# jl6017/AutoURDF

Measured on AMD Instinct MI355X. Metric: registered frames/sec (N=4096 pts, K=20 clusters), higher is better.
Workload: dtype f32

## Files before the change

autourdf_amd/csrc/nn_l1.h:

```cpp
#pragma once
#include <type_traits>
#include "creg_dev.h"

namespace creg {

constexpr int NN_TCH = 4096;
constexpr int NN_BLOCK = 512;
typedef float nn_f2 __attribute__((ext_vector_type(2)));

struct NnEpilogueNone {
    __device__ __forceinline__ void finish(int, int, float, float*) const {}
    __device__ __forceinline__ void shift(int) {}
};

template <int QW, typename IdxT, typename Epi>
__device__ __forceinline__ void nn_l1_block(
    const float* A, int na, int sa, const float* B, int nb, int sb,
    float* __restrict__ dA, IdxT* __restrict__ iA, float* __restrict__ dB, IdxT* __restrict__ iB,
    int blocksA, Epi& epi, int bx) {
    extern __shared__ __attribute__((aligned(16))) char smem_raw[];
    float* sX = (float*)smem_raw;
    __shared__ float s_part[NN_BLOCK / 64];
    const int tid = threadIdx.x, lane = tid & 63;
    const int wave = __builtin_amdgcn_readfirstlane(tid >> 6);
// ... 73 lines not shown
#pragma unroll
        for (int e = 3; e >= 0; --e) {
            const int j = bgrp[u] + 64 * e;
            const float d = l1_dist(qx[u], qy[u], qz[u], rx[u][e], ry[u][e], rz[u][e]);
            if (bgrp[u] >= 0 && j < nt && d == best[u]) bi = j;
        }
        float v = best[u]; int i = bi;
        wave_argmin_fast(v, i);
        if (lane == u) { mv = v; mi = i; mqx = qx[u]; mqy = qy[u]; mqz = qz[u]; }
    }
    if (lane < QW && q0 + lane < nq) {
        if (dO) { dO[q0 + lane] = mv; iO[q0 + lane] = (IdxT)mi; }
        if constexpr (!std::is_same<Epi, NnEpilogueNone>::value) {
            float tx, ty, tz;
            if (in_lds) { tx = sX[mi]; ty = sX[padded0 + mi]; tz = sX[2 * padded0 + mi]; }
            else { const float* p = T + (size_t)mi * st; tx = p[0]; ty = p[1]; tz = p[2]; }
            epi(dir, q0 + lane, mi, mv, mqx, mqy, mqz, tx, ty, tz, acc);
        }
    }
    if constexpr (!std::is_same<Epi, NnEpilogueNone>::value) {
        acc = wave_sum_fast(acc);
        if (lane == 0) s_part[wave] = acc;
        __syncthreads();
        if (tid == 0) {
            float s = 0.f;
#pragma unroll
            for (int w = 0; w < NN_BLOCK / 64; ++w) s += s_part[w];
            epi.finish(dir, blk, s, nullptr);
        }
    }
}

struct NnBlocks { const float4* ts4; const float* tbox; int nblk; const int* nblk_dev; };

template <int NB, int PPL, typename Epi, bool STOP = false, bool NBDEV = false>
__device__ __forceinline__ void nn_l1_block_pruned(const float* Q, int nq, int sq, NnBlocks tb, int dir, Epi& epi, int blk,
                                                   const int* stop_flag = nullptr, const float* T = nullptr, int st = 0) {
    constexpr int QW = 4;
    int stop = 0;
    if constexpr (STOP) stop = *stop_flag;
    __shared__ float s_partp[NN_BLOCK / 64];
    const int tid = threadIdx.x, lane = tid & 63;
    const int wave = __builtin_amdgcn_readfirstlane(tid >> 6);
    const int q0 = (blk * (NN_BLOCK / 64) + wave) * QW;
    int nblk = tb.nblk;
    if constexpr (NBDEV) nblk = *tb.nblk_dev;
    float lox[NB], loy[NB], loz[NB], hix[NB], hiy[NB], hiz[NB];
#pragma unroll
    for (int g = 0; g < NB; ++g) {
        const float* bx = tb.tbox + (NBDEV ? 64 * g + lane : min(64 * g + lane, nblk - 1));
        constexpr int BP = 64 * NB;
        lox[g] = bx[0]; loy[g] = bx[BP]; loz[g] = bx[2 * BP]; hix[g] = bx[3 * BP]; hiy[g] = bx[4 * BP]; hiz[g] = bx[5 * BP];
    }
    float qx[QW], qy[QW], qz[QW], lb[QW][NB], bd[QW], tx[QW], ty[QW], tz[QW], wb[QW];
    int bi[QW];
    unsigned long long pend[QW][NB];
#pragma unroll
    for (int u = 0; u < QW; ++u) {
        const int qi = min(q0 + u, nq - 1);
        qx[u] = Q[(size_t)qi * sq]; qy[u] = Q[(size_t)qi * sq + 1]; qz[u] = Q[(size_t)qi * sq + 2];
    }
    if constexpr (STOP || NBDEV) {
        stop = __builtin_amdgcn_readfirstlane(stop); nblk = __builtin_amdgcn_readfirstlane(nblk);
#pragma unroll
        for (int u = 0; u < QW; ++u) {
            qx[u] = __int_as_float(__builtin_amdgcn_readfirstlane(__float_as_int(qx[u])));
            qy[u] = __int_as_float(__builtin_amdgcn_readfirstlane(__float_as_int(qy[u])));
            qz[u] = __int_as_float(__builtin_amdgcn_readfirstlane(__float_as_int(qz[u])));
        }
    }
#pragma unroll
    for (int u = 0; u < QW; ++u) {
        float lm = INFINITY;
#pragma unroll
        for (int g = 0; g < NB; ++g) {
            const float ex = fmaxf(fmaxf(lox[g] - qx[u], qx[u] - hix[g]), 0.f);
            const float ey = fmaxf(fmaxf(loy[g] - qy[u], qy[u] - hiy[g]), 0.f);
            const float ez = fmaxf(fmaxf(loz[g] - qz[u], qz[u] - hiz[g]), 0.f);
            const float bound = (ex + ey) + ez;
            lb[u][g] = 64 * g + lane < nblk ? bound : INFINITY;
            lm = __builtin_fminf(lm, lb[u][g]);
        }
        const float m = wave_min_fast(lm);
        bool found = false;
#pragma unroll
        for (int g = 0; g < NB; ++g) {
            const unsigned long long f = __ballot(lb[u][g] == m && 64 * g + lane < nblk);
            pend[u][g] = (!found && f) ? (f & (~f + 1ull)) : 0ull;
            found = found || f != 0ull;
        }
        if (!found) pend[u][0] = 1ull;
        bd[u] = INFINITY; bi[u] = 0x7fffffff; tx[u] = ty[u] = tz[u] = 0.f; wb[u] = INFINITY;
    }
    if (stop) return;
    bool more = true;
    while (more) {
        int b[QW];
        bool act[QW];
#pragma unroll
        for (int u = 0; u < QW; ++u) {
            b[u] = 0; act[u] = false;
#pragma unroll
            for (int g = NB - 1; g >= 0; --g)
                if (pend[u][g]) { b[u] = 64 * g + __builtin_ctzll(pend[u][g]); act[u] = true; }
        }
        float4 v1[QW];
        if constexpr (PPL == 1) {
#pragma unroll
            for (int u = 0; u < QW; ++u) v1[u] = tb.ts4[(size_t)b[u] * 64 + lane];
        }
        more = false;
#pragma unroll
        for (int u = 0; u < QW; ++u) {
            if (act[u]) {
                float4 v[PPL];
                if constexpr (PPL == 1) v[0] = v1[u];
                else {
#pragma unroll
                    for (int k = 0; k < PPL; ++k) v[k] = tb.ts4[((size_t)b[u] * PPL + k) * 64 + lane];
                }
#pragma unroll
                for (int g = 0; g < NB; ++g)
                    if ((b[u] >> 6) == g && lane == (b[u] & 63)) lb[u][g] = INFINITY;
                if constexpr (PPL > 1) {
                    unsigned long long key = ((unsigned long long)__float_as_uint(bd[u]) << 32) | (unsigned)bi[u];
#pragma unroll
                    for (int k = 0; k < PPL; ++k) {
                        const float d = l1_dist(qx[u], qy[u], qz[u], v[k].x, v[k].y, v[k].z);
                        const unsigned long long kk = ((unsigned long long)__float_as_uint(d) << 32) | (unsigned)__float_as_int(v[k].w);
                        key = kk < key ? kk : key;
                    }
                    bd[u] = __uint_as_float((unsigned)(key >> 32)); bi[u] = (int)(unsigned)key;
                } else {
#pragma unroll
                    for (int k = 0; k < PPL; ++k) {
                        const float d = l1_dist(qx[u], qy[u], qz[u], v[k].x, v[k].y, v[k].z);
                        const int oi = __float_as_int(v[k].w);
                        const unsigned long long key = ((unsigned long long)__float_as_uint(bd[u]) << 32) | (unsigned)bi[u];
                        const unsigned long long kk = ((unsigned long long)__float_as_uint(d) << 32) | (unsigned)oi;
                        const bool take = kk < key;
                        bd[u] = take ? d : bd[u]; bi[u] = take ? oi : bi[u];
                        tx[u] = take ? v[k].x : tx[u]; ty[u] = take ? v[k].y : ty[u]; tz[u] = take ? v[k].z : tz[u];
                    }
                }
                wb[u] = wave_min_fast(bd[u]);
#pragma unroll
                for (int g = 0; g < NB; ++g) {
                    pend[u][g] = __ballot(lb[u][g] <= wb[u] && lb[u][g] < INFINITY);
                    more |= pend[u][g] != 0ull;
                }
            }
        }
    }
    float acc = 0.f, mv = 0.f, mqx = 0.f, mqy = 0.f, mqz = 0.f, mtx = 0.f, mty = 0.f, mtz = 0.f;
    int mi = 0;
#pragma unroll
    for (int u = 0; u < QW; ++u) {
        const int i = wave_min_fast(bd[u] == wb[u] ? bi[u] : 0x7fffffff);
        const unsigned long long win = __ballot(bd[u] == wb[u] && bi[u] == i);
        const int src = win ? __builtin_ctzll(win) : 0;
        const float fx = __int_as_float(__builtin_amdgcn_readlane(__float_as_int(tx[u]), src));
        const float fy = __int_as_float(__builtin_amdgcn_readlane(__float_as_int(ty[u]), src));
        const float fz = __int_as_float(__builtin_amdgcn_readlane(__float_as_int(tz[u]), src));
        if (lane == u) { mv = wb[u]; mi = i; mqx = qx[u]; mqy = qy[u]; mqz = qz[u]; mtx = fx; mty = fy; mtz = fz; }
    }
    if constexpr (PPL > 1) {
        if (lane < QW && q0 + lane < nq && mi != 0x7fffffff) { const float* p = T + (size_t)mi * st; mtx = p[0]; mty = p[1]; mtz = p[2]; }
    }
    if (lane < QW && q0 + lane < nq) epi(dir, q0 + lane, mi, mv, mqx, mqy, mqz, mtx, mty, mtz, acc);
    acc = wave_sum_fast(acc);
    if (lane == 0) s_partp[wave] = acc;
    __syncthreads();
    if (tid == 0) {
        float s = 0.f;
#pragma unroll
        for (int w = 0; w < NN_BLOCK / 64; ++w) s += s_partp[w];
        epi.finish(dir, blk, s, nullptr);
    }
}

__device__ __forceinline__ float row_min16(float v) {
    asm("s_nop 4\n\t"
        "v_min_f32_dpp %0, %0, %0 quad_perm:[1,0,3,2] row_mask:0xf bank_mask:0xf\n\ts_nop 1\n\t"
        "v_min_f32_dpp %0, %0, %0 quad_perm:[2,3,0,1] row_mask:0xf bank_mask:0xf\n\ts_nop 1\n\t"
        "v_min_f32_dpp %0, %0, %0 row_half_mirror row_mask:0xf bank_mask:0xf\n\ts_nop 1\n\t"
        "v_min_f32_dpp %0, %0, %0 row_mirror row_mask:0xf bank_mask:0xf\n\ts_nop 1"
        : "+v"(v));
    return v;
}
__device__ __forceinline__ float row_max16(float v) {
    asm("s_nop 4\n\t"
        "v_max_f32_dpp %0, %0, %0 quad_perm:[1,0,3,2] row_mask:0xf bank_mask:0xf\n\ts_nop 1\n\t"
        "v_max_f32_dpp %0, %0, %0 quad_perm:[2,3,0,1] row_mask:0xf bank_mask:0xf\n\ts_nop 1\n\t"
        "v_max_f32_dpp %0, %0, %0 row_half_mirror row_mask:0xf bank_mask:0xf\n\ts_nop 1\n\t"
        "v_max_f32_dpp %0, %0, %0 row_mirror row_mask:0xf bank_mask:0xf\n\ts_nop 1"
        : "+v"(v));
    return v;
}
__device__ __forceinline__ float row_sum16_f(float v) {
    CREG_DPP_STEP(v, 0xB1, 0xF);
    CREG_DPP_STEP(v, 0x4E, 0xF);
    CREG_DPP_STEP(v, 0x141, 0xF);
    CREG_DPP_STEP(v, 0x140, 0xF);
    return v;
}
__device__ __forceinline__ unsigned long long key_min_rows(unsigned long long k) {
    {   const auto hi = __builtin_amdgcn_permlane16_swap((unsigned)(k >> 32), (unsigned)(k >> 32), false, false);
        const auto lo = __builtin_amdgcn_permlane16_swap((unsigned)k, (unsigned)k, false, false);
        const unsigned long long a = ((unsigned long long)hi[0] << 32) | lo[0], b = ((unsigned long long)hi[1] << 32) | lo[1];
        k = a < b ? a : b; }
    {   const auto hi = __builtin_amdgcn_permlane32_swap((unsigned)(k >> 32), (unsigned)(k >> 32), false, false);
        const auto lo = __builtin_amdgcn_permlane32_swap((unsigned)k, (unsigned)k, false, false);
        const unsigned long long a = ((unsigned long long)hi[0] << 32) | lo[0], b = ((unsigned long long)hi[1] << 32) | lo[1];
        k = a < b ? a : b; }
    return k;
}
#ifdef CREG_NN_STATS
__device__ unsigned long long g_nn_stats[8];
#define NN_STAT(i, v) do { if (lane == 0) atomicAdd(&g_nn_stats[i], (unsigned long long)(v)); } while (0)
#else
#define NN_STAT(i, v) do { } while (0)
#endif
#ifdef CREG_NN_WAVE_STAMPS
struct NnWaveRec { unsigned long long t0, t1, t2, t3; int visits, cands, dir, blk; };
constexpr unsigned NN_WAVE_CAP = 1u << 19, NN_WAVE_SHARDS = 256, NN_WAVE_PER = NN_WAVE_CAP / NN_WAVE_SHARDS;
__device__ NnWaveRec g_nn_wave[NN_WAVE_CAP];
__device__ unsigned g_nn_wave_n[NN_WAVE_SHARDS * 32];
#define NN_WSTAMP(...) __VA_ARGS__
#else
#define NN_WSTAMP(...)
#endif
constexpr int NN_ROWQ = 16;
#ifndef NN_ROW_FIRST
#define NN_ROW_FIRST 2
#endif
#ifndef NN_ROW_BATCH
#define NN_ROW_BATCH 3
#endif
#ifndef NN_ROWS_BLOCK
#define NN_ROWS_BLOCK 256
#endif
constexpr int NN_ROW_SLOTS = (NN_ROWS_BLOCK / 64) * NN_ROWQ;

template <int NB, typename Epi, bool NBDEV, bool NQDEV>
__device__ __forceinline__ void nn_l1_rows(const float4* __restrict__ qs4, int nqblk, const int* nqblk_dev, int nqblk_host, NnBlocks tb, int dir, Epi& epi, int blk,
                                           const int* stop_flag, const float* __restrict__ T, float* __restrict__ lossp) {
    const int tid = threadIdx.x, lane = tid & 63, q = lane & 15, g = lane >> 4;
    const int wave = __builtin_amdgcn_readfirstlane(tid >> 6);
    const int grp = blk * (NN_ROWS_BLOCK / 64) + wave;
    if (grp >= 4 * nqblk_host) return;
    NN_WSTAMP(const unsigned long long ws_t0 = (unsigned long long)wall_clock64(); unsigned long long ws_t1 = 0, ws_t2 = 0; int ws_vis = 0, ws_cand = 0;)
    int stop = *stop_flag;
    int nblk = tb.nblk;
    if constexpr (NBDEV) nblk = *tb.nblk_dev;
    if constexpr (NQDEV) nqblk = *nqblk_dev;
// ... 175 lines not shown
```

autourdf_amd/csrc/train_backward.hip:

```cpp
#include <cmath>
#include <cstddef>
#include <cstring>
#include "train_dev.h"

namespace creg {

__device__ __forceinline__ TrainState advance_state(const TrainState& S, float loss, const Hyper& hy, double bc1, float bc2_sqrt) {
    TrainState N = S;
    const bool improved = loss < S.min_loss;
    N.last_loss = loss;
    N.epochs_run = S.epochs_run + 1;
    const int count = improved ? 0 : S.count + 1;
    N.min_loss = improved ? loss : S.min_loss;
    N.best_epoch = improved ? S.epochs_run : S.best_epoch;
    N.count = count;
    N.stopped = (!improved && count > hy.stop) ? 1 : S.stopped;
    if (!N.stopped) {
        N.step = S.step + 1;
        N.step_size = (float)(S.lr / bc1);
        N.bc2_sqrt = bc2_sqrt;
        const double cur = (double)loss;
        if (cur < S.sched_best * (1.0 - 1e-4)) { N.sched_best = cur; N.sched_bad = 0; }
        else N.sched_bad = S.sched_bad + 1;
        if (N.sched_bad > hy.patience) {
            const double nl = fmax(S.lr * (double)hy.factor, 0.0);
            if (S.lr - nl > 1e-8) N.lr = nl;
            N.sched_bad = 0;
        }
    }
    return N;
}

constexpr int GC_QMAX = 3;
__device__ __forceinline__ void gradc_role(const Dims& D, const Ws& W, int epoch, int nbx, int nby, int k) {
    __shared__ float red[4][14];
    __shared__ float s_loss;
    __shared__ float s_go[16];
    const int tid = threadIdx.x, lane = tid & 63, wv = tid >> 6;
    const TrainState S = W.state[epoch & 1];
    const int b0 = W.off[k], e0 = W.off[k + 1];
    const Hyper hy = *W.hyper;
    float a = tid < nbx ? W.lossp_x[tid] : 0.f, b = tid < nby ? W.lossp_y[tid] : 0.f;
    const float m2v = W.m2[16 * k + (tid & 15)];
    float sv[16];
#pragma unroll
    for (int i = 0; i < 16; ++i) sv[i] = W.head_save[16 * k + i];
    const float* h2cur = (epoch & 1) ? W.h2[1] : W.h2[0];
    float w3v[GC_QMAX][8], h2v[GC_QMAX];
#pragma unroll
    for (int q = 0; q < GC_QMAX; ++q) {
        const int o = min(q * 256 + tid, D.H2 - 1);
        const bool isA = o < D.HA;
        const float* Pc = (epoch & 1) ? W.P1 : W.P;
        const float* wb = isA ? Pc + D.oW3A + o : Pc + D.oW3B + (o - D.HA);
        const int stride = isA ? D.HA : D.HB, nj = isA ? D.OA : D.OB;
#pragma unroll
        for (int j = 0; j < 8; ++j) w3v[q][j] = wb[(size_t)min(j, nj - 1) * stride];
        h2v[q] = h2cur[(size_t)k * D.H2 + o];
    }
    asm volatile("" :: "v"(a), "v"(b), "v"(m2v), "v"(sv[0]), "v"(sv[1]), "v"(sv[2]), "v"(sv[3]), "v"(sv[4]), "v"(sv[5]), "v"(sv[6]), "v"(sv[7]),
                 "v"(sv[8]), "v"(sv[9]), "v"(sv[10]), "v"(sv[11]), "v"(sv[12]), "v"(sv[13]), "v"(sv[14]), "v"(sv[15]), "v"(b0), "v"(e0), "v"(hy.lr));
#pragma unroll
    for (int q = 0; q < GC_QMAX; ++q)
        asm volatile("" :: "v"(h2v[q]), "v"(w3v[q][0]), "v"(w3v[q][1]), "v"(w3v[q][2]), "v"(w3v[q][3]), "v"(w3v[q][4]), "v"(w3v[q][5]), "v"(w3v[q][6]),
                     "v"(w3v[q][7]));
    if (S.stopped) {
        if (k == 0 && tid == 0) {
            TrainState E = S; E.stopped = 1;
            W.state[(epoch + 1) & 1] = E;
        }
        return;
    }
    const int n_first = min(b0 + tid, D.NP - 1);
    const float4 p_first = W.pts4[n_first];
    const int4 c_first = W.cnt4[n_first];
    const int s_first = W.sgn_x[n_first];
    const float4 pr_first = W.pred4[n_first];
    for (int i = tid + 256; i < nbx; i += 256) a += W.lossp_x[i];
    for (int i = tid + 256; i < nby; i += 256) b += W.lossp_y[i];
    a = wave_sum_fast(a); b = wave_sum_fast(b);
    if (lane == 0) { red[wv][0] = a; red[wv][1] = b; }
    __syncthreads();
    if (tid == 0) {
        const float sa = ((red[0][0] + red[1][0]) + red[2][0]) + red[3][0];
        const float sb = ((red[0][1] + red[1][1]) + red[2][1]) + red[3][1];
        s_loss = sa / (float)D.NP + sb / (float)D.NT;
    }
    __syncthreads();
    const float loss = s_loss;
    TrainState N = advance_state(S, loss, hy, S.next_bc1, S.next_bc2s);
    const bool improved = loss < S.min_loss;
    if (improved) {
        for (int n = b0 + tid; n < e0; n += 256) {
            const float4 p = (n == b0 + tid) ? pr_first : W.pred4[n];
            W.best_pred[3 * (size_t)n] = p.x; W.best_pred[3 * (size_t)n + 1] = p.y; W.best_pred[3 * (size_t)n + 2] = p.z;
        }
        if (tid < 16) W.best_m[16 * k + tid] = m2v;
    }
    if (k == 0 && tid == 0) {
        N.next_bc1 = W.bc1[min(N.step + 1, D.epochs)];
        N.next_bc2s = W.bc2s[min(N.step + 1, D.epochs)];
        W.state[(epoch + 1) & 1] = N;
        W.loss_hist[S.epochs_run] = loss;
        W.lr_hist[S.epochs_run] = (float)S.lr;
        W.result[0] = N.min_loss; W.result[1] = (float)N.epochs_run; W.result[2] = (float)N.lr; W.result[3] = (float)N.best_epoch;
    }
    if (N.stopped) return;
    const float gx = 1.0f / (float)D.NP, gy = 1.0f / (float)D.NT;
    float acc[12];
#pragma unroll
    for (int i = 0; i < 12; ++i) acc[i] = 0.f;
    for (int n = b0 + tid; n < e0; n += 256) {
// ... 34 lines not shown
            float gu[4];
            quat_to_matrix_vjp(sv, G, gu);
            const float nrm = sv[4];
            if (nrm > 1e-12f) {
                const float dot = sv[0] * gu[0] + sv[1] * gu[1] + sv[2] * gu[2] + sv[3] * gu[3];
#pragma unroll
                for (int i = 0; i < 4; ++i) go[4 + i] = (gu[i] - sv[i] * dot) / nrm;
            } else {
#pragma unroll
                for (int i = 0; i < 4; ++i) go[4 + i] = gu[i] / 1e-12f;
            }
        } else {
            float gdq[8];
            dq_to_se3_vjp(sv, G, gt, gdq);
            for (int i = 0; i < 8; ++i) go[4 + i] = gdq[i];
        }
        for (int i = 0; i < 12; ++i) { W.g_out[16 * k + i] = go[i]; s_go[i] = go[i]; }
    }
    __syncthreads();
#pragma unroll
    for (int q = 0; q < GC_QMAX; ++q) {
        const int o = q * 256 + tid;
        if (o < D.H2) {
            const bool isA = o < D.HA;
            const int nj = isA ? D.OA : D.OB, gofs = isA ? 0 : 4;
            float sum = 0.f;
#pragma unroll
            for (int j = 0; j < 8; ++j) if (j < nj) sum = fmaf(s_go[gofs + j], w3v[q][j], sum);
            W.g_h2[(size_t)k * D.H2 + o] = sum * act_grad(h2v[q], D.slope);
        }
    }
}

__global__ __launch_bounds__(256) void k_gradc(Dims D, Ws W0, int epoch, int nbx, int nby, size_t bstride) {
    asm volatile("" :: "s"(W0.P), "s"(W0.P1), "s"(W0.h2[0]), "s"(W0.h2[1]), "s"(W0.head_save), "s"(W0.m2), "s"(W0.gm2), "s"(W0.pts4), "s"(W0.pred4),
                 "s"(W0.sgn_x), "s"(W0.cnt4), "s"(W0.lossp_x), "s"(W0.lossp_y), "s"(W0.g_out), "s"(W0.g_h2), "s"(W0.state), "s"(W0.bc1), "s"(W0.bc2s),
                 "s"(W0.best_m), "s"(W0.best_pred), "s"(W0.loss_hist), "s"(W0.lr_hist), "s"(W0.result), "s"(W0.off), "s"(W0.hyper),
                 "s"(D.rot), "s"(D.K), "s"(D.H2), "s"(D.HA), "s"(D.HB), "s"(D.OA), "s"(D.OB), "s"(D.NP), "s"(D.NT), "s"(D.epochs), "s"(D.slope),
                 "s"(D.oW3A), "s"(D.oW3B), "s"(epoch), "s"(nbx), "s"(nby), "s"(bstride));
    const Ws W = ws_shift(W0, blockIdx.z * bstride);
    gradc_role(D, W, epoch, nbx, nby, blockIdx.x);
}

__device__ __forceinline__ float adam_value(float p, float& mm, float& vv, float g, float step_size, float bc2_sqrt) {
    const float b1w = (float)(1.0 - 0.9), b2 = 0.999f, b2w = (float)(1.0 - 0.999);
    mm = mm + b1w * (g - mm);
    vv = vv * b2 + (b2w * g) * g;
    const float denom = sqrtf(vv) / bc2_sqrt + 1e-8f;
    return p + (-step_size * mm) / denom;
}

#ifdef CREG_BD_STAMPS
struct BdStamps {
    unsigned long long first[256], endB[256], endD[256], startB[256], startD[256];
    unsigned long long phase[2][8], blocks[2];
    int armed;
};
__device__ BdStamps g_bd_st;
#endif
constexpr int BD_THREADS = 512;
constexpr int B2_THREADS = BD_THREADS;
constexpr int B2_WAVES = B2_THREADS / 64;
constexpr int B2_CB = 16;
constexpr int B2_RB = 32;
__host__ __device__ inline int b2_smem_floats(int K, int IN, int H2) {
    return B2_WAVES * B2_RB * B2_CB + K * IN + 2 * K * B2_CB + H2 * B2_CB;
}
__device__ __forceinline__ float row_sum16(float v) {
    CREG_DPP_STEP(v, 0xB1, 0xF);
    CREG_DPP_STEP(v, 0x4E, 0xF);
    CREG_DPP_STEP(v, 0x141, 0xF);
    CREG_DPP_STEP(v, 0x140, 0xF);
    return v;
}
// ... 264 lines not shown
__global__ __launch_bounds__(BD_THREADS, 4) void k_bd(Dims D, Ws W0, int epoch, size_t bstride, int nz) {
    extern __shared__ __attribute__((aligned(16))) char smem[];
#ifdef CREG_BD_STAMPS
    const unsigned long long bd_entry = wall_clock64();
#else
    const unsigned long long bd_entry = 0;
#endif
#ifndef CREG_BD_NO_TOUCH
    asm volatile("" :: "s"(W0.P), "s"(W0.P1), "s"(W0.AM), "s"(W0.AV), "s"(W0.enc), "s"(W0.x1[0]), "s"(W0.x1[1]), "s"(W0.h2[0]), "s"(W0.h2[1]),
                 "s"(W0.g_out), "s"(W0.g_h2), "s"(W0.state), "s"(D.K), "s"(D.KP), "s"(D.IN), "s"(D.H), "s"(D.H2), "s"(D.HA), "s"(D.HB), "s"(D.OA),
                 "s"(D.OB), "s"(D.oW1), "s"(D.ob1), "s"(D.oW2), "s"(D.ob2), "s"(D.oW3A), "s"(D.ob3A), "s"(D.oW3B), "s"(D.ob3B), "s"(D.NPAR),
                 "s"(D.slope), "s"(epoch), "s"(bstride), "s"(nz));
#endif
    const int nB = D.H / B2_CB, nD = dw_blocks(D);
    int i = blockIdx.x;
    const bool roleB = i < nB * nz;
    if (!roleB) i -= nB * nz;
    const int n = roleB ? nB : nD, z = i / n, blk = i - z * n;
    const Ws W = ws_shift(W0, (size_t)z * bstride);
#ifdef CREG_BD_ONLY
    if ((CREG_BD_ONLY == 1) != roleB) return;
#endif
    if (roleB) bwd2_role<KW, X>(D, W, epoch, blk, (float*)smem, bd_entry);
    else dw_role(D, W, epoch, blk, bd_entry);
}
constexpr int BD_K_MAX_6D_512 = 193;
constexpr int BD_LDS_MAX = 160 * 1024;
static int bd_lds_bytes(const Dims& D) { return (int)sizeof(float) * b2_smem_floats(D.K, D.IN, D.H2); }
bool backward_fits(const Dims& D) {
    if (D.rot == ROT_6D && D.H == 512 && D.K > BD_K_MAX_6D_512) return false;
    return D.K * D.IN / 4 <= 8 * BD_THREADS && bd_lds_bytes(D) <= BD_LDS_MAX && D.H2 % 32 == 0 && D.H % B2_CB == 0 && D.H2 <= 256 * GC_QMAX;
}
void launch_gradc(const Dims& D, const Slice& S, size_t bstride, int epoch, hipStream_t s) {
    hipLaunchKernelGGL(k_gradc, dim3(D.K, 1, S.nz), dim3(256), 0, s, D, S.W, epoch, D.nbx, D.nby, bstride);
}
template <typename F>
static void by_bd(const Dims& D, F f) {
    by_nc(D.H, [&](auto nc) {
        constexpr int NC = decltype(nc)::value;
        if (D.IN > 64) f(k_bd<NC, 12 * NC, true>);
        else if (D.HA) f(k_bd<NC, 12 * NC>);
        else f(k_bd<NC, 8 * NC>);
    });
}
int bd_raise_lds(const Dims& D) {
    hipError_t e = hipSuccess;
    by_bd(D, [&](auto kern) { e = hipFuncSetAttribute((const void*)kern, hipFuncAttributeMaxDynamicSharedMemorySize, BD_LDS_MAX); });
    if (e != hipSuccess) {
        set_error("creg_train_plan_create: cannot raise the dynamic LDS limit of k_bd: %s", hipGetErrorString(e));
        return CREG_EHIP;
    }
    return CREG_OK;
}
void launch_bd(const Dims& D, const Slice& S, size_t bstride, int epoch, hipStream_t s) {
    const int per = D.H / B2_CB + dw_blocks(D);
    by_bd(D, [&](auto kern) { hipLaunchKernelGGL(kern, dim3(per * S.nz), dim3(BD_THREADS), bd_lds_bytes(D), s, D, S.W, epoch, bstride, S.nz); });
}

int bd_stamps_arm(bool on) {
#ifdef CREG_BD_STAMPS
    static BdStamps z;
    if (on) {
        memset(&z, 0, sizeof(z)); memset(z.first, 0xff, sizeof(z.first)); memset(z.startB, 0xff, sizeof(z.startB)); memset(z.startD, 0xff, sizeof(z.startD));
        z.armed = 1;
        CREG_HIP(hipMemcpyToSymbol(HIP_SYMBOL(g_bd_st), &z, sizeof(z)));
    } else {
        z.armed = 0;
// ... 32 lines not shown
```

autourdf_amd/csrc/train_dev.h:

```cpp
#pragma once
#include <type_traits>
#include "creg_common.h"
#include "creg_dev.h"

namespace creg {

struct Dims {
    int rot, K, KP, IN, H, HA, HB, H2, OA, OB, NP, NT, epochs;
    float slope;
    int oW1, ob1, oW2, ob2, oW3A, ob3A, oW3B, ob3B, NPAR;
    int nbx, nby;
    int nyb;
    int npb;
    int ppl;
    int nbt, nbp;
    int rows;
};

constexpr int PS_MAXB = 512;
constexpr int YS_CHUNK = 16384;

struct Hyper {
    float lr, factor;
    int patience, stop;
};

struct TrainState {
    double lr, sched_best;
    int sched_bad, count, stopped, step;
    float min_loss;
    int epochs_run, best_epoch;
    float step_size, bc2_sqrt;
    float last_loss;
    float next_bc2s;
    double next_bc1;
};

struct Ws {
    float *P, *P1, *AM, *AV;
    float *pose_in, *enc, *x1[2], *h2[2], *head_save, *m2, *gm2;
    float4 *pts4, *y4, *pred4, *ys4, *psl4, *ps4;
    float *ybox, *pbox;
    int* sb;
    int* sgn_x;
    int4* cnt4;
    float *lossp_x, *lossp_y;
    float *g_out, *g_h2;
    TrainState* state;
    double* bc1;
    float* bc2s;
// ... 75 lines not shown
```

autourdf_amd/csrc/train_engine.hip:

```cpp
#include <chrono>
#include <cstdlib>
#include <cstring>
#include <memory>
#include <vector>
#include "train_dev.h"
#include "nn_l1.h"

namespace creg {

constexpr int CHAINS_MAX = 8;

struct Plan {
    creg_train_shape shape{};
    Dims D{};
    Ws W{};
    ParamMap pm[10] = {};
    int np = 0;
    int B = 1;
    size_t bstride = 0;
    int branches = 1;
    hipGraphExec_t gexec = nullptr;
    bool graph_ready = false;
    int graph_epochs = 0;
    bool chain_streams = false;
// ... 28 lines not shown

static bool make_dims(const creg_train_shape* s, Dims* D) {
    if (!s || s->rot < 0 || s->rot > 3 || s->k < 1 || s->k > 256 || (s->hidden != 64 && s->hidden != 128 && s->hidden != 256 && s->hidden != 512) || s->epochs < 1 || s->n_pred < 1 || s->n_tgt < 1 || s->n_pred >= (1ll << 31) ||
        s->n_tgt >= (1ll << 31))
        return false;
    memset(D, 0, sizeof(*D));
    D->rot = s->rot; D->K = s->k; D->KP = (s->k + 19) / 20 * 20; D->H = s->hidden; D->NP = (int)s->n_pred; D->NT = (int)s->n_tgt; D->epochs = s->epochs;
    if (s->rot == ROT_Q) { D->IN = 56; D->HA = D->H / 2; D->HB = D->H; D->OA = 3; D->OB = 4; D->slope = 0.01f; }
    else if (s->rot == ROT_DQ) { D->IN = 64; D->HA = 0; D->HB = D->H; D->OA = 0; D->OB = 8; D->slope = 0.f; }
    else if (s->rot == ROT_6D) { D->IN = 72; D->HA = D->H / 2; D->HB = D->H; D->OA = 3; D->OB = 6; D->slope = 0.01f; }
    else { D->IN = 48; D->HA = D->H / 2; D->HB = D->H; D->OA = 3; D->OB = 3; D->slope = 0.01f; }
    D->H2 = D->HA + D->HB;
    if (!backward_fits(*D)) return false;
    int o = 0;
    D->oW1 = o; o += D->H * D->IN; D->ob1 = o; o += D->H;
    D->oW2 = o; o += D->H2 * D->H; D->ob2 = o; o += D->H2;
    D->oW3A = o; o += D->OA * D->HA; D->ob3A = o; o += D->OA;
    D->oW3B = o; o += D->OB * D->HB; D->ob3B = o; o += D->OB;
    D->NPAR = o;
    const NnGrid g = nn_grid(D->NP, D->NT, true, true, 4);
    D->nbx = g.blocksA; D->nby = g.blocksB;
    const bool rows_fit = D->NT <= YS_CHUNK && D->NP < 65535 && (D->NP + 63) / 64 + D->K <= PS_MAXB && g.qw == 4;
    const char* rows_env = getenv("CREG_NN_ROWS");
    const bool rows_pays = D->NT > 64 * 64;
    D->rows = s->nn_search == 0 && rows_fit && (rows_env ? rows_env[0] == '1' : rows_pays);
    D->ppl = (D->rows || D->NT <= 64 * 64) ? 1 : 4;
    const int BS = 64 * D->ppl;
    D->nyb = (s->nn_search != 1 && D->NT <= 4 * YS_CHUNK && g.qw == 4) ? (D->NT + BS - 1) / BS : 0;
    D->npb = (D->nyb && D->NP < 65535 && (D->NP + BS - 1) / BS + D->K <= PS_MAXB) ? (D->NP + BS - 1) / BS + D->K : 0;
    const int nt = (D->nyb + 63) / 64, np = (D->npb + 63) / 64;
    D->nbt = nt <= 1 ? 1 : (nt <= 2 ? 2 : 4);
    D->nbp = np <= 2 ? 2 : (np <= 3 ? 3 : (np <= 4 ? 4 : (np <= 5 ? 5 : (np <= 6 ? 6 : 8))));
    if (D->rows) { D->nbx = 4 * D->npb; D->nby = 4 * D->nyb; }
    return true;
}

static size_t carve(const Dims& D, char* base, Ws* W) {
    size_t o = 0;
    auto take = [&](size_t bytes) -> char* { char* r = base ? base + o : nullptr; o = align_up(o + bytes, 256); return r; };
    const size_t f = sizeof(float);
    Ws w;
    w.P = (float*)take(f * D.NPAR); w.P1 = (float*)take(f * D.NPAR); w.AM = (float*)take(f * D.NPAR); w.AV = (float*)take(f * D.NPAR);
    w.pose_in = (float*)take(f * POSE_IN * D.K); w.enc = (float*)take(f * D.K * D.IN);
    w.x1[0] = (float*)take(f * D.KP * D.H); w.x1[1] = (float*)take(f * D.KP * D.H);
    w.h2[0] = (float*)take(f * D.KP * D.H2); w.h2[1] = (float*)take(f * D.KP * D.H2); w.head_save = (float*)take(f * 16 * D.K);
    w.m2 = (float*)take(f * 16 * D.K); w.gm2 = (float*)take(f * 16 * D.K);
    w.pts4 = (float4*)take(sizeof(float4) * D.NP); w.y4 = (float4*)take(sizeof(float4) * D.NT);
    w.pred4 = (float4*)take(sizeof(float4) * D.NP);
    const size_t bs = 64 * (size_t)D.ppl;
    w.ys4 = (float4*)take(sizeof(float4) * bs * (D.nyb ? D.nyb : 1)); w.ybox = (float*)take(f * 6 * 64 * D.nbt);
    w.psl4 = (float4*)take(sizeof(float4) * bs * (D.npb ? D.npb : 1)); w.ps4 = (float4*)take(sizeof(float4) * bs * (D.npb ? D.npb : 1));
    w.pbox = (float*)take(f * 6 * 64 * D.nbp); w.sb = (int*)take(sizeof(int) * (D.K + 1));
    w.sgn_x = (int*)take(sizeof(int) * D.NP);
    w.cnt4 = (int4*)take(sizeof(int4) * D.NP);
    w.lossp_x = (float*)take(f * D.nbx); w.lossp_y = (float*)take(f * D.nby);
    w.g_out = (float*)take(f * 16 * D.KP); w.g_h2 = (float*)take(f * D.KP * D.H2);
    w.state = (TrainState*)take(sizeof(TrainState) * 2);
    w.bc1 = (double*)take(sizeof(double) * (D.epochs + 1)); w.bc2s = (float*)take(f * (D.epochs + 1));
    w.best_m = (float*)take(f * 16 * D.K); w.best_pred = (float*)take(f * 3 * D.NP);
    w.loss_hist = (float*)take(f * D.epochs); w.lr_hist = (float*)take(f * D.epochs); w.result = (float*)take(f * 4);
    w.off = (int*)take(sizeof(int) * (D.K + 1)); w.hyper = (Hyper*)take(sizeof(Hyper));
    w.ysum = (unsigned long long*)take(sizeof(unsigned long long) * 4);
    if (W) *W = w;
    return o;
}
constexpr int NKERN = 5;
// ... 406 lines not shown
```

autourdf_amd/csrc/train_nn.hip:

```cpp
#include <type_traits>
#include <vector>
#include "train_dev.h"
#include "nn_l1.h"

namespace creg {

struct EngineEpi {
    int* sgn_x; int4* cnt4; float* lossp_x; float* lossp_y;
    size_t bstride;
    const int* stopped;
    __device__ __forceinline__ void shift(int z) {
        const size_t b = (size_t)z * bstride;
        sgn_x = (int*)((char*)sgn_x + b); cnt4 = (int4*)((char*)cnt4 + b);
        lossp_x = (float*)((char*)lossp_x + b); lossp_y = (float*)((char*)lossp_y + b);
        stopped = (const int*)((const char*)stopped + b);
    }
    __device__ __forceinline__ void operator()(int dir, int q, int idx, float d, float qx, float qy, float qz,
                                               float tx, float ty, float tz, float& acc) const {
        if (dir == 0) {
            sgn_x[q] = (qx > tx ? 1 : 0) | (qy > ty ? 2 : 0) | (qz > tz ? 4 : 0);
        } else {
            atomicAdd(&cnt4[idx].x, (qx > tx) ? -1 : 1);
            atomicAdd(&cnt4[idx].y, (qy > ty) ? -1 : 1);
            atomicAdd(&cnt4[idx].z, (qz > tz) ? -1 : 1);
        }
        acc += d;
    }
    __device__ __forceinline__ void finish(int dir, int blk, float s, float*) const { (dir == 0 ? lossp_x : lossp_y)[blk] = s; }
};

template <bool P1, int PPL, int NBT, int NBP>
__global__ __launch_bounds__(NN_BLOCK) void k_nn_plan(const float* A, int na, const float* B, int nb, int blocksA,
                                                      int blocksB, EngineEpi epi, NnBlocks yb, NnBlocks pb, size_t zstride) {
    asm volatile("" :: "s"(A), "s"(na), "s"(B), "s"(nb), "s"(blocksA), "s"(blocksB), "s"(epi.sgn_x), "s"(epi.cnt4), "s"(epi.lossp_x), "s"(epi.lossp_y),
                 "s"(epi.bstride), "s"(epi.stopped), "s"(yb.ts4), "s"(yb.tbox), "s"(yb.nblk), "s"(pb.ts4), "s"(pb.tbox), "s"(pb.nblk_dev), "s"(zstride));
    const int nz = gridDim.x / (blocksA + blocksB);
    int i = blockIdx.x, z, bx;
    if (i < blocksB * nz) { z = i / blocksB; bx = blocksA + (i - z * blocksB); }
    else { i -= blocksB * nz; z = i / blocksA; bx = i - z * blocksA; }
    const size_t zb = z * zstride;
    A = (const float*)((const char*)A + zb);
    B = (const float*)((const char*)B + zb);
    yb.ts4 = (const float4*)((const char*)yb.ts4 + zb);
    yb.tbox = (const float*)((const char*)yb.tbox + zb);
    epi.shift(z);
    if (bx < blocksA) nn_l1_block_pruned<NBT, PPL, EngineEpi, true, false>(A, na, 4, yb, 0, epi, bx, epi.stopped, B, 4);
    else if constexpr (P1) {
        pb.ts4 = (const float4*)((const char*)pb.ts4 + zb);
        pb.tbox = (const float*)((const char*)pb.tbox + zb);
        pb.nblk_dev = (const int*)((const char*)pb.nblk_dev + zb);
        nn_l1_block_pruned<NBP, PPL, EngineEpi, true, true>(B, nb, 4, pb, 1, epi, bx - blocksA, epi.stopped, A, 4);
    } else nn_l1_block<4, int, EngineEpi>(A, na, 4, B, nb, 4, nullptr, nullptr, nullptr, nullptr, blocksA, epi, bx);
}

template <int NBT, int NBP>
__global__ __launch_bounds__(NN_ROWS_BLOCK) void k_nn_rows(const float* A, const float* B, int blocksA, int blocksB, EngineEpi epi, NnBlocks yb, NnBlocks pb,
                                                      size_t zstride) {
    asm volatile("" :: "s"(A), "s"(B), "s"(blocksA), "s"(blocksB), "s"(epi.sgn_x), "s"(epi.cnt4), "s"(epi.lossp_x), "s"(epi.lossp_y),
                 "s"(epi.bstride), "s"(epi.stopped), "s"(yb.ts4), "s"(yb.tbox), "s"(yb.nblk), "s"(pb.ts4), "s"(pb.tbox), "s"(pb.nblk_dev), "s"(zstride));
    const int nz = gridDim.x / (blocksA + blocksB);
    int i = blockIdx.x, z, bx;
    if (i < blocksB * nz) { z = i / blocksB; bx = blocksA + (i - z * blocksB); }
    else { i -= blocksB * nz; z = i / blocksA; bx = i - z * blocksA; }
    const size_t zb = z * zstride;
    A = (const float*)((const char*)A + zb);
    B = (const float*)((const char*)B + zb);
    yb.ts4 = (const float4*)((const char*)yb.ts4 + zb);
    yb.tbox = (const float*)((const char*)yb.tbox + zb);
    pb.ts4 = (const float4*)((const char*)pb.ts4 + zb);
    pb.tbox = (const float*)((const char*)pb.tbox + zb);
    pb.nblk_dev = (const int*)((const char*)pb.nblk_dev + zb);
    epi.shift(z);
    if (bx < blocksA) nn_l1_rows<NBT, EngineEpi, false, true>(pb.ts4, 0, pb.nblk_dev, pb.nblk, yb, 0, epi, bx, epi.stopped, B, epi.lossp_x);
    else nn_l1_rows<NBP, EngineEpi, true, false>(yb.ts4, yb.nblk, nullptr, yb.nblk, pb, 1, epi, bx - blocksA, epi.stopped, A, epi.lossp_y);
}
template <typename F>
static void by_boxes(int nbt, int nbp, F f) {
    by_value<1, 2, 4>(nbt, [&](auto t) { by_value<2, 3, 4, 5, 6, 8>(nbp, [&](auto p) { f(t, p); }); });
}

void launch_nn(const Dims& D, const Slice& S, size_t bstride, int par, hipStream_t s) {
    const Ws& W = S.W;
    const int nz = S.nz;
    const EngineEpi epi{W.sgn_x, W.cnt4, W.lossp_x, W.lossp_y, bstride, &W.state[par].stopped};
    if (D.rows) {
        const NnBlocks yb{W.ys4, W.ybox, D.nyb, nullptr}, pb{W.ps4, W.pbox, D.npb, W.sb + D.K};
        const int blocksA = cdiv(64 * D.npb, NN_ROW_SLOTS), blocksB = cdiv(64 * D.nyb, NN_ROW_SLOTS);
        const dim3 grid((blocksA + blocksB) * nz);
        by_boxes(D.nbt, D.nbp, [&](auto nbt, auto nbp) {
            hipLaunchKernelGGL((k_nn_rows<decltype(nbt)::value, decltype(nbp)::value>), grid, dim3(NN_ROWS_BLOCK), 0, s, (const float*)W.pred4, (const float*)W.y4,
                               blocksA, blocksB, epi, yb, pb, bstride);
        });
    } else if (D.nyb) {
        const NnGrid g = nn_grid(D.NP, D.NT, true, true, 4);
        const NnBlocks yb{W.ys4, W.ybox, D.nyb, nullptr}, pb{W.ps4, W.pbox, 0, W.sb + D.K};
        const dim3 grid((g.blocksA + g.blocksB) * nz);
        auto go = [&](auto kern, int smem) {
            hipLaunchKernelGGL(kern, grid, dim3(NN_BLOCK), smem, s, (const float*)W.pred4, D.NP, (const float*)W.y4, D.NT,
                               g.blocksA, g.blocksB, epi, yb, pb, bstride);
        };
        by_value<1, 4>(D.ppl, [&](auto ppl) {
            by_boxes(D.nbt, D.nbp, [&](auto nbt, auto nbp) {
                constexpr int PPL = decltype(ppl)::value, NBT = decltype(nbt)::value, NBP = decltype(nbp)::value;
                if constexpr (NBP == 2) if (!D.npb) { go(k_nn_plan<false, PPL, NBT, 2>, g.smem); return; }
                go(k_nn_plan<true, PPL, NBT, NBP>, 0);
            });
        });
    } else {
        launch_nn_l1<int>((const float*)W.pred4, D.NP, 4, (const float*)W.y4, D.NT, 4, nullptr, nullptr, nullptr, nullptr,
                          true, true, epi, s, nz, bstride, 4);
    }
}

}
using namespace creg;

#ifdef CREG_NN_STATS
extern "C" int creg_debug_nn_stats(unsigned long long* out8, int reset) {
    CREG_HIP(hipMemcpyFromSymbol(out8, HIP_SYMBOL(creg::g_nn_stats), sizeof(unsigned long long) * 8));
    if (reset) { unsigned long long z[8] = {0}; CREG_HIP(hipMemcpyToSymbol(HIP_SYMBOL(creg::g_nn_stats), z, sizeof(z))); }
    return CREG_OK;
}
#endif
// ... 24 lines not shown
```

Before: 166.5.

## Add slot-ordered NN query kernel with per-point distance write and fused gradc loss sum

Adds a new k_nn_slot path in which each wave takes its four queries in spatial slot order from the other cloud's sorted block storage. Queries that are spatially close therefore tend to visit the same target block, and the block is loaded once when all active queries agree. Each query's distance is written back into the .w of pred4/y4 rather than reduced per block into lossp partials. k_gradc then rebuilds the loss sums itself with DPP block partials, which drops the block reduction and __syncthreads from the NN kernel. The path is on by default, with an env var to opt out, and only applies for ppl==1 with both clouds boxed and small enough. It risks extra global writes and more complex control flow.

Result: slower. 137.9 (-17.2%).

```diff
diff --git a/autourdf_amd/csrc/nn_l1.h b/autourdf_amd/csrc/nn_l1.h
--- a/autourdf_amd/csrc/nn_l1.h
+++ b/autourdf_amd/csrc/nn_l1.h
@@ -129,17 +129,31 @@
 }
 
 struct NnBlocks { const float4* ts4; const float* tbox; int nblk; const int* nblk_dev; };
-
-template <int NB, int PPL, typename Epi, bool STOP = false, bool NBDEV = false>
+#ifdef CREG_NN_STATS
+__device__ unsigned long long g_nn_stats[8];
+#define NN_STAT(i, v) do { if (lane == 0) atomicAdd(&g_nn_stats[i], (unsigned long long)(v)); } while (0)
+#else
+#define NN_STAT(i, v) do { } while (0)
+#endif
+
+template <int NB, int PPL, typename Epi, bool STOP = false, bool NBDEV = false, int SLOTW = 0, bool NQDEV = false>
 __device__ __forceinline__ void nn_l1_block_pruned(const float* Q, int nq, int sq, NnBlocks tb, int dir, Epi& epi, int blk,
-                                                   const int* stop_flag = nullptr, const float* T = nullptr, int st = 0) {
+                                                   const int* stop_flag = nullptr, const float* T = nullptr, int st = 0,
+                                                   const float4* __restrict__ qs4 = nullptr, int nqblk = 0, const int* nqblk_dev = nullptr) {
     constexpr int QW = 4;
+    constexpr bool SLOT = SLOTW > 0;
+    static_assert(!SLOT || (PPL == 1 && STOP), "slot-order queries: one point per lane, with the stop flag");
     int stop = 0;
     if constexpr (STOP) stop = *stop_flag;
     __shared__ float s_partp[NN_BLOCK / 64];
     const int tid = threadIdx.x, lane = tid & 63;
     const int wave = __builtin_amdgcn_readfirstlane(tid >> 6);
-    const int q0 = (blk * (NN_BLOCK / 64) + wave) * QW;
+    const int q0 = (blk * (SLOT ? SLOTW : NN_BLOCK / 64) + wave) * QW;
+    float4 qv = make_float4(0.f, 0.f, 0.f, 0.f);
+    if constexpr (SLOT) {
+        if constexpr (NQDEV) nqblk = *nqblk_dev;
+        qv = qs4[q0 + (lane & 3)];
+    }
     int nblk = tb.nblk;
     if constexpr (NBDEV) nblk = *tb.nblk_dev;
     float lox[NB], loy[NB], loz[NB], hix[NB], hiy[NB], hiz[NB];
@@ -151,13 +165,33 @@
     }
     float qx[QW], qy[QW], qz[QW], lb[QW][NB], bd[QW], tx[QW], ty[QW], tz[QW], wb[QW];
     int bi[QW];
+    unsigned vmask = 0xFu;
+    bool lvalid = true;
     unsigned long long pend[QW][NB];
+    if constexpr (SLOT) {
+        asm volatile("" :: "v"(qv.x), "v"(qv.y), "v"(qv.z), "v"(qv.w), "v"(nblk));
+#pragma unroll
+        for (int g = 0; g < NB; ++g) asm volatile("" :: "v"(lox[g]), "v"(loy[g]), "v"(loz[g]), "v"(hix[g]), "v"(hiy[g]), "v"(hiz[g]));
+        stop = __builtin_amdgcn_readfirstlane(stop); nqblk = __builtin_amdgcn_readfirstlane(nqblk);
+        lvalid = q0 + (lane & 3) < 64 * nqblk && __float_as_int(qv.w) != 0x7fffffff;
+        vmask = (unsigned)__ballot(lvalid) & 0xFu;
+        if (stop || !vmask) return;
+        nblk = __builtin_amdgcn_readfirstlane(nblk);
+#pragma unroll
+        for (int u = 0; u < QW; ++u) {
+            qx[u] = __int_as_float(__builtin_amdgcn_readlane(__float_as_int(qv.x), u));
+            qy[u] = __int_as_float(__builtin_amdgcn_readlane(__float_as_int(qv.y), u));
+            qz[u] = __int_as_float(__builtin_amdgcn_readlane(__float_as_int(qv.z), u));
+        }
+        NN_STAT(0 + 4 * dir, 1); NN_STAT(3 + 4 * dir, __builtin_popcount(vmask));
+    } else {
 #pragma unroll
     for (int u = 0; u < QW; ++u) {
         const int qi = min(q0 + u, nq - 1);
         qx[u] = Q[(size_t)qi * sq]; qy[u] = Q[(size_t)qi * sq + 1]; qz[u] = Q[(size_t)qi * sq + 2];
     }
-    if constexpr (STOP || NBDEV) {
+    }
+    if constexpr (!SLOT && (STOP || NBDEV)) {
         stop = __builtin_amdgcn_readfirstlane(stop); nblk = __builtin_amdgcn_readfirstlane(nblk);
 #pragma unroll
         for (int u = 0; u < QW; ++u) {
@@ -187,9 +221,20 @@
             found = found || f != 0ull;
         }
         if (!found) pend[u][0] = 1ull;
+        if constexpr (SLOT) {
+            if (!((vmask >> u) & 1u)) {
+#pragma unroll
+                for (int g = 0; g < NB; ++g) pend[u][g] = 0ull;
+            }
+        }
         bd[u] = INFINITY; bi[u] = 0x7fffffff; tx[u] = ty[u] = tz[u] = 0.f; wb[u] = INFINITY;
     }
-    if (stop) return;
+    if constexpr (!SLOT) {
+        if (stop) return;
+#ifdef CREG_NN_STATS
+        if (q0 < nq) { NN_STAT(0 + 4 * dir, 1); NN_STAT(3 + 4 * dir, min(QW, nq - q0)); }
+#endif
+    }
     bool more = true;
     while (more) {
         int b[QW];
@@ -202,7 +247,25 @@
                 if (pend[u][g]) { b[u] = 64 * g + __builtin_ctzll(pend[u][g]); act[u] = true; }
         }
         float4 v1[QW];
-        if constexpr (PPL == 1) {
+        if constexpr (SLOT) {
+            int bs = 0;
+            bool first = true, same = true;
+#pragma unroll
+            for (int u = 0; u < QW; ++u)
+                if (act[u]) { same = same && (first || b[u] == bs); if (first) { bs = b[u]; first = false; } }
+            NN_STAT(1 + 4 * dir, 1);
+            if (same) {
+                const float4 v = tb.ts4[(size_t)bs * 64 + lane];
+#pragma unroll
+                for (int u = 0; u < QW; ++u) v1[u] = v;
+            } else {
+#pragma unroll
+                for (int u = 0; u < QW; ++u) v1[u] = tb.ts4[(size_t)(act[u] ? b[u] : bs) * 64 + lane];
+            }
+        } else if constexpr (PPL == 1) {
+#ifdef CREG_NN_STATS
+            if (q0 < nq) NN_STAT(1 + 4 * dir, 1);
+#endif
 #pragma unroll
             for (int u = 0; u < QW; ++u) v1[u] = tb.ts4[(size_t)b[u] * 64 + lane];
         }
@@ -210,6 +273,9 @@
 #pragma unroll
         for (int u = 0; u < QW; ++u) {
             if (act[u]) {
+#ifdef CREG_NN_STATS
+                if (SLOT || q0 + u < nq) NN_STAT(2 + 4 * dir, 1);
+#endif
                 float4 v[PPL];
                 if constexpr (PPL == 1) v[0] = v1[u];
                 else {
@@ -264,15 +330,19 @@
     if constexpr (PPL > 1) {
         if (lane < QW && q0 + lane < nq && mi != 0x7fffffff) { const float* p = T + (size_t)mi * st; mtx = p[0]; mty = p[1]; mtz = p[2]; }
     }
-    if (lane < QW && q0 + lane < nq) epi(dir, q0 + lane, mi, mv, mqx, mqy, mqz, mtx, mty, mtz, acc);
-    acc = wave_sum_fast(acc);
-    if (lane == 0) s_partp[wave] = acc;
-    __syncthreads();
-    if (tid == 0) {
-        float s = 0.f;
-#pragma unroll
-        for (int w = 0; w < NN_BLOCK / 64; ++w) s += s_partp[w];
-        epi.finish(dir, blk, s, nullptr);
+    if constexpr (SLOT) {
+        if (lane < QW && lvalid) epi(dir, __float_as_int(qv.w), mi, mv, mqx, mqy, mqz, mtx, mty, mtz, acc);
+    } else {
+        if (lane < QW && q0 + lane < nq) epi(dir, q0 + lane, mi, mv, mqx, mqy, mqz, mtx, mty, mtz, acc);
+        acc = wave_sum_fast(acc);
+        if (lane == 0) s_partp[wave] = acc;
+        __syncthreads();
+        if (tid == 0) {
+            float s = 0.f;
+#pragma unroll
+            for (int w = 0; w < NN_BLOCK / 64; ++w) s += s_partp[w];
+            epi.finish(dir, blk, s, nullptr);
+        }
     }
 }
 
@@ -312,12 +382,6 @@
         k = a < b ? a : b; }
     return k;
 }
-#ifdef CREG_NN_STATS
-__device__ unsigned long long g_nn_stats[8];
-#define NN_STAT(i, v) do { if (lane == 0) atomicAdd(&g_nn_stats[i], (unsigned long long)(v)); } while (0)
-#else
-#define NN_STAT(i, v) do { } while (0)
-#endif
 #ifdef CREG_NN_WAVE_STAMPS
 struct NnWaveRec { unsigned long long t0, t1, t2, t3; int visits, cands, dir, blk; };
 constexpr unsigned NN_WAVE_CAP = 1u << 19, NN_WAVE_SHARDS = 256, NN_WAVE_PER = NN_WAVE_CAP / NN_WAVE_SHARDS;
diff --git a/autourdf_amd/csrc/train_backward.hip b/autourdf_amd/csrc/train_backward.hip
--- a/autourdf_amd/csrc/train_backward.hip
+++ b/autourdf_amd/csrc/train_backward.hip
@@ -32,15 +32,37 @@
 }
 
 constexpr int GC_QMAX = 3;
+constexpr int GC_PMAX = 2 * 8 * GC_LQ;
+__device__ __forceinline__ float gc_block_partials(float v) {
+    CREG_DPP_STEP(v, 0xB1, 0xF);
+    CREG_DPP_STEP(v, 0x4E, 0xF);
+    float c = v;
+#pragma unroll
+    for (int i = 0; i < 3; ++i) c = __int_as_float(__builtin_amdgcn_update_dpp(0, __float_as_int(c), 0x114, 0xF, 0xF, false)) + v;
+    float e = __int_as_float(__builtin_amdgcn_update_dpp(0, __float_as_int(c), 0x142, 0xA, 0xF, false)) + v;
+#pragma unroll
+    for (int i = 0; i < 3; ++i) e = __int_as_float(__builtin_amdgcn_update_dpp(0, __float_as_int(e), 0x114, 0xF, 0xF, false)) + v;
+    return e;
+}
+template <bool SQ>
 __device__ __forceinline__ void gradc_role(const Dims& D, const Ws& W, int epoch, int nbx, int nby, int k) {
     __shared__ float red[4][14];
+    __shared__ float s_lp[SQ ? GC_PMAX : 1];
     __shared__ float s_loss;
     __shared__ float s_go[16];
     const int tid = threadIdx.x, lane = tid & 63, wv = tid >> 6;
     const TrainState S = W.state[epoch & 1];
     const int b0 = W.off[k], e0 = W.off[k + 1];
     const Hyper hy = *W.hyper;
-    float a = tid < nbx ? W.lossp_x[tid] : 0.f, b = tid < nby ? W.lossp_y[tid] : 0.f;
+    float a = 0.f, b = 0.f;
+    float dqx[GC_LQ], dqy[GC_LQ];
+    if constexpr (SQ) {
+#pragma unroll
+        for (int j = 0; j < GC_LQ; ++j) {
+            dqx[j] = W.pred4[min(256 * j + tid, D.NP - 1)].w;
+            dqy[j] = W.y4[min(256 * j + tid, D.NT - 1)].w;
+        }
+    } else { a = tid < nbx ? W.lossp_x[tid] : 0.f; b = tid < nby ? W.lossp_y[tid] : 0.f; }
     const float m2v = W.m2[16 * k + (tid & 15)];
     float sv[16];
 #pragma unroll
@@ -57,6 +79,10 @@
 #pragma unroll
         for (int j = 0; j < 8; ++j) w3v[q][j] = wb[(size_t)min(j, nj - 1) * stride];
         h2v[q] = h2cur[(size_t)k * D.H2 + o];
+    }
+    if constexpr (SQ) {
+#pragma unroll
+        for (int j = 0; j < GC_LQ; ++j) asm volatile("" :: "v"(dqx[j]), "v"(dqy[j]));
     }
     asm volatile("" :: "v"(a), "v"(b), "v"(m2v), "v"(sv[0]), "v"(sv[1]), "v"(sv[2]), "v"(sv[3]), "v"(sv[4]), "v"(sv[5]), "v"(sv[6]), "v"(sv[7]),
                  "v"(sv[8]), "v"(sv[9]), "v"(sv[10]), "v"(sv[11]), "v"(sv[12]), "v"(sv[13]), "v"(sv[14]), "v"(sv[15]), "v"(b0), "v"(e0), "v"(hy.lr));
@@ -76,8 +102,19 @@
     const int4 c_first = W.cnt4[n_first];
     const int s_first = W.sgn_x[n_first];
     const float4 pr_first = W.pred4[n_first];
+    if constexpr (SQ) {
+#pragma unroll
+        for (int j = 0; j < GC_LQ; ++j) {
+            const float px = gc_block_partials(256 * j + tid < D.NP ? dqx[j] : 0.f), py = gc_block_partials(256 * j + tid < D.NT ? dqy[j] : 0.f);
+            if ((lane & 31) == 31) { s_lp[8 * j + (tid >> 5)] = px; s_lp[GC_PMAX / 2 + 8 * j + (tid >> 5)] = py; }
+        }
+        __syncthreads();
+        for (int i = tid; i < nbx; i += 256) a += s_lp[i];
+        for (int i = tid; i < nby; i += 256) b += s_lp[GC_PMAX / 2 + i];
+    } else {
     for (int i = tid + 256; i < nbx; i += 256) a += W.lossp_x[i];
     for (int i = tid + 256; i < nby; i += 256) b += W.lossp_y[i];
+    }
     a = wave_sum_fast(a); b = wave_sum_fast(b);
     if (lane == 0) { red[wv][0] = a; red[wv][1] = b; }
     __syncthreads();
@@ -178,6 +215,7 @@
     }
 }
 
+template <bool SQ>
 __global__ __launch_bounds__(256) void k_gradc(Dims D, Ws W0, int epoch, int nbx, int nby, size_t bstride) {
     asm volatile("" :: "s"(W0.P), "s"(W0.P1), "s"(W0.h2[0]), "s"(W0.h2[1]), "s"(W0.head_save), "s"(W0.m2), "s"(W0.gm2), "s"(W0.pts4), "s"(W0.pred4),
                  "s"(W0.sgn_x), "s"(W0.cnt4), "s"(W0.lossp_x), "s"(W0.lossp_y), "s"(W0.g_out), "s"(W0.g_h2), "s"(W0.state), "s"(W0.bc1), "s"(W0.bc2s),
@@ -185,7 +223,7 @@
                  "s"(D.rot), "s"(D.K), "s"(D.H2), "s"(D.HA), "s"(D.HB), "s"(D.OA), "s"(D.OB), "s"(D.NP), "s"(D.NT), "s"(D.epochs), "s"(D.slope),
                  "s"(D.oW3A), "s"(D.oW3B), "s"(epoch), "s"(nbx), "s"(nby), "s"(bstride));
     const Ws W = ws_shift(W0, blockIdx.z * bstride);
-    gradc_role(D, W, epoch, nbx, nby, blockIdx.x);
+    gradc_role<SQ>(D, W, epoch, nbx, nby, blockIdx.x);
 }
 
 __device__ __forceinline__ float adam_value(float p, float& mm, float& vv, float g, float step_size, float bc2_sqrt) {
@@ -516,7 +554,8 @@
     return D.K * D.IN / 4 <= 8 * BD_THREADS && bd_lds_bytes(D) <= BD_LDS_MAX && D.H2 % 32 == 0 && D.H % B2_CB == 0 && D.H2 <= 256 * GC_QMAX;
 }
 void launch_gradc(const Dims& D, const Slice& S, size_t bstride, int epoch, hipStream_t s) {
-    hipLaunchKernelGGL(k_gradc, dim3(D.K, 1, S.nz), dim3(256), 0, s, D, S.W, epoch, D.nbx, D.nby, bstride);
+    if (D.slotq) hipLaunchKernelGGL(k_gradc<true>, dim3(D.K, 1, S.nz), dim3(256), 0, s, D, S.W, epoch, D.nbx, D.nby, bstride);
+    else hipLaunchKernelGGL(k_gradc<false>, dim3(D.K, 1, S.nz), dim3(256), 0, s, D, S.W, epoch, D.nbx, D.nby, bstride);
 }
 template <typename F>
 static void by_bd(const Dims& D, F f) {
diff --git a/autourdf_amd/csrc/train_dev.h b/autourdf_amd/csrc/train_dev.h
--- a/autourdf_amd/csrc/train_dev.h
+++ b/autourdf_amd/csrc/train_dev.h
@@ -15,7 +15,9 @@
     int ppl;
     int nbt, nbp;
     int rows;
+    int slotq;
 };
+constexpr int GC_LQ = 16;
 
 constexpr int PS_MAXB = 512;
 constexpr int YS_CHUNK = 16384;
diff --git a/autourdf_amd/csrc/train_engine.hip b/autourdf_amd/csrc/train_engine.hip
--- a/autourdf_amd/csrc/train_engine.hip
+++ b/autourdf_amd/csrc/train_engine.hip
@@ -84,6 +84,8 @@
     D->nbt = nt <= 1 ? 1 : (nt <= 2 ? 2 : 4);
     D->nbp = np <= 2 ? 2 : (np <= 3 ? 3 : (np <= 4 ? 4 : (np <= 5 ? 5 : (np <= 6 ? 6 : 8))));
     if (D->rows) { D->nbx = 4 * D->npb; D->nby = 4 * D->nyb; }
+    const char* slot_env = getenv("CREG_NN_SLOTQ");
+    D->slotq = !D->rows && D->nyb && D->npb && D->ppl == 1 && D->NP <= 256 * GC_LQ && D->NT <= 256 * GC_LQ && !(slot_env && slot_env[0] == '0');
     return true;
 }
 
diff --git a/autourdf_amd/csrc/train_nn.hip b/autourdf_amd/csrc/train_nn.hip
--- a/autourdf_amd/csrc/train_nn.hip
+++ b/autourdf_amd/csrc/train_nn.hip
@@ -28,6 +28,15 @@
     }
     __device__ __forceinline__ void finish(int dir, int blk, float s, float*) const { (dir == 0 ? lossp_x : lossp_y)[blk] = s; }
 };
+struct EngineEpiSlot {
+    EngineEpi e;
+    float4 *dist_x, *dist_y;
+    __device__ __forceinline__ void operator()(int dir, int q, int idx, float d, float qx, float qy, float qz,
+                                               float tx, float ty, float tz, float& acc) const {
+        e(dir, q, idx, d, qx, qy, qz, tx, ty, tz, acc);
+        (dir == 0 ? dist_x : dist_y)[q].w = d;
+    }
+};
 
 template <bool P1, int PPL, int NBT, int NBP>
 __global__ __launch_bounds__(NN_BLOCK) void k_nn_plan(const float* A, int na, const float* B, int nb, int blocksA,
@@ -51,6 +60,32 @@
         pb.nblk_dev = (const int*)((const char*)pb.nblk_dev + zb);
         nn_l1_block_pruned<NBP, PPL, EngineEpi, true, true>(B, nb, 4, pb, 1, epi, bx - blocksA, epi.stopped, A, 4);
     } else nn_l1_block<4, int, EngineEpi>(A, na, 4, B, nb, 4, nullptr, nullptr, nullptr, nullptr, blocksA, epi, bx);
+}
+
+#ifndef NN_SLOT_BLOCK
+#define NN_SLOT_BLOCK 256
+#endif
+constexpr int NN_SLOT_WAVES = NN_SLOT_BLOCK / 64;
+template <int NBT, int NBP>
+__global__ __launch_bounds__(NN_SLOT_BLOCK) void k_nn_slot(float4* A, float4* B, int blocksA, int blocksB, EngineEpi epi, NnBlocks yb, NnBlocks pb, size_t zstride) {
+    asm volatile("" :: "s"(A), "s"(B), "s"(blocksA), "s"(blocksB), "s"(epi.sgn_x), "s"(epi.cnt4), "s"(epi.bstride), "s"(epi.stopped),
+                 "s"(yb.ts4), "s"(yb.tbox), "s"(yb.nblk), "s"(pb.ts4), "s"(pb.tbox), "s"(pb.nblk), "s"(pb.nblk_dev), "s"(zstride));
+    const int nz = gridDim.x / (blocksA + blocksB);
+    int i = blockIdx.x, z, bx;
+    if (i < blocksB * nz) { z = i / blocksB; bx = blocksA + (i - z * blocksB); }
+    else { i -= blocksB * nz; z = i / blocksA; bx = i - z * blocksA; }
+    const size_t zb = z * zstride;
+    yb.ts4 = (const float4*)((const char*)yb.ts4 + zb);
+    yb.tbox = (const float*)((const char*)yb.tbox + zb);
+    pb.ts4 = (const float4*)((const char*)pb.ts4 + zb);
+    pb.tbox = (const float*)((const char*)pb.tbox + zb);
+    pb.nblk_dev = (const int*)((const char*)pb.nblk_dev + zb);
+    epi.shift(z);
+    EngineEpiSlot es{epi, (float4*)((char*)A + zb), (float4*)((char*)B + zb)};
+    if (bx < blocksA)
+        nn_l1_block_pruned<NBT, 1, EngineEpiSlot, true, false, NN_SLOT_WAVES, true>(nullptr, 0, 4, yb, 0, es, bx, epi.stopped, nullptr, 4, pb.ts4, 0, pb.nblk_dev);
+    else
+        nn_l1_block_pruned<NBP, 1, EngineEpiSlot, true, true, NN_SLOT_WAVES, false>(nullptr, 0, 4, pb, 1, es, bx - blocksA, epi.stopped, nullptr, 4, yb.ts4, yb.nblk, nullptr);
 }
 
 template <int NBT, int NBP>
@@ -89,6 +124,14 @@
         const dim3 grid((blocksA + blocksB) * nz);
         by_boxes(D.nbt, D.nbp, [&](auto nbt, auto nbp) {
             hipLaunchKernelGGL((k_nn_rows<decltype(nbt)::value, decltype(nbp)::value>), grid, dim3(NN_ROWS_BLOCK), 0, s, (const float*)W.pred4, (const float*)W.y4,
+                               blocksA, blocksB, epi, yb, pb, bstride);
+        });
+    } else if (D.slotq) {
+        const NnBlocks yb{W.ys4, W.ybox, D.nyb, nullptr}, pb{W.ps4, W.pbox, D.npb, W.sb + D.K};
+        const int blocksA = 16 * D.npb / NN_SLOT_WAVES, blocksB = 16 * D.nyb / NN_SLOT_WAVES;
+        const dim3 grid((blocksA + blocksB) * nz);
+        by_boxes(D.nbt, D.nbp, [&](auto nbt, auto nbp) {
+            hipLaunchKernelGGL((k_nn_slot<decltype(nbt)::value, decltype(nbp)::value>), grid, dim3(NN_SLOT_BLOCK), 0, s, W.pred4, W.y4,
                                blocksA, blocksB, epi, yb, pb, bstride);
         });
     } else if (D.nyb) {
```
